# nka77/DAHiTra

Hardware: AMD Instinct MI355X
Metric: image-pairs/s (256x256) train step, 1/2/4/8 MI355X + CPU ref (higher is better)
Workload: dtype bf16; 1 GPU; LEVIR-CD 256x256 synthetic pairs, base_transformer_pos_s4, bf16, batch 32 per GPU (global 32), fwd+focal+bwd+allreduce+AdamW; net_G=base_transformer_pos_s4, global_batch=32, img_size=256, parallelism=dp1, hip_graph=True, step_form=one graph (AdamW inside), attn_dtype=bf16

## Files before the change

### dahitra_amd/csrc/conv_wgrad.hip

```cpp
#include "common.h"

namespace {

constexpr int TH = 8, TW = 16;
static inline int co_tile(int Cout) { return Cout <= 16 ? 16 : (Cout <= 32 ? 32 : 64); }

struct WgArgs {
    const void* x;
    const void* dy;
    float* part;
    int N, H, W, Cin, OH, OW, Cout, pad;
    int tilesX, tilesY, splitk, groups, npix, in_npix;
    int ci_tiles;
    int CinPitch;
    int dil;
    int CoutUse;
    int direct;
    const float* in_scale;
    const float* in_shift;
    int in_groups;
    int phase_mode;
    int no_xcd_remap;
    const void* dyt_y;
    const float* dytoef;
    int dyt_groups;
    long x_split;
};

constexpr int lds_pitch(int row_bytes) { return ((row_bytes / 32) & 1) ? row_bytes : row_bytes + 32; }

union F8 {
    s16x8 v;
    s16x4 h[2];
// ... 432 lines not shown
    bool okij[NI][4];
#pragma unroll
    for (int i = 0; i < NI; ++i)
#pragma unroll
        for (int j = 0; j < 4; ++j)
            okij[i][j] = WCI ? (cob + i * 16 + j < p.CoutUse && cib < p.Cin) : (cob + j < p.CoutUse && cib + i * 16 < p.Cin);
    if (p.direct == 2) {
#pragma unroll
        for (int t = 0; t < TAPS; ++t)
#pragma unroll
            for (int i = 0; i < NI; ++i)
#pragma unroll
                for (int j = 0; j < 4; ++j)
                    if (okij[i][j]) out[t * tstride + j * p.Cin + i * istep] += acc[t][i][j];
    } else {
#pragma unroll
        for (int t = 0; t < TAPS; ++t)
#pragma unroll
            for (int i = 0; i < NI; ++i)
#pragma unroll
                for (int j = 0; j < 4; ++j)
                    if (okij[i][j]) out[t * tstride + j * p.Cin + i * istep] = acc[t][i][j];
    }
}
template <typename T, int KS, int STRIDE, int IT, bool TR, int DIL, int CTT, int CIG, bool DYT = false>
__global__ __launch_bounds__(256 * CIG) void conv_wgrad_kernel(WgArgs p) {
    extern __shared__ __attribute__((aligned(16))) unsigned char smem[];
    wg_body<T, KS, STRIDE, IT, TR, DIL, CTT, CIG, DYT>(p, blockIdx.x, blockIdx.y, gridDim.x, gridDim.y, blockIdx.z, smem);
}
constexpr int WS_MAXJ = 16;
struct WsMulti {
    int njobs;
    int first[WS_MAXJ + 1];
    WgArgs a[WS_MAXJ];
};
static_assert(sizeof(WsMulti) <= 4096, "the kernel argument block");
template <typename T, int KS, int STRIDE, int IT, bool TR, int DIL, int CTT, int CIG>
__global__ __launch_bounds__(256 * CIG) void conv_wgrad_multi_kernel(WsMulti m) {
    extern __shared__ __attribute__((aligned(16))) unsigned char smem[];
    int j = 0;
    while (j + 1 < m.njobs && (int)blockIdx.x >= m.first[j + 1]) ++j;
    const WgArgs p = m.a[j];
    const int nbx = ((p.CoutUse + CTT - 1) / CTT) * p.ci_tiles, local = (int)blockIdx.x - m.first[j];
    if (local >= nbx * p.splitk) return;
    wg_body<T, KS, STRIDE, IT, TR, DIL, CTT, CIG, false>(p, local % nbx, local / nbx, nbx, p.splitk, 0, smem);
}

static inline int wgrad_reduce_epb(int I) { return (I & 3) == 0 ? 128 : 32; }
__device__ __forceinline__ void wgrad_reduce_block(const float* __restrict__ part, int splitk, int taps, int Oslab, int O,
                                                   int I, float* __restrict__ dw, int accumulate, long block, float (*red)[132]) {
    const long n = (long)O * I * taps;
    const int lane = threadIdx.x & 31, ph = threadIdx.x >> 5;
    const bool vec = (I & 3) == 0;
    const long i = vec ? (block * 32 + lane) * 4 : block * 32 + lane;
    float acc[4] = {0.f, 0.f, 0.f, 0.f};
    int tap = 0, ci = 0, o = 0;
    if (i < n) {
        ci = (int)(i % I);
        o = (int)((i / I) % O);
        tap = (int)(i / ((long)I * O));
        const size_t slab = (size_t)taps * Oslab * I;
        const float* src = part + ((size_t)tap * Oslab + o) * I + ci;
        if (vec) {
            float4 a0 = make_float4(0.f, 0.f, 0.f, 0.f), a1 = a0, a2 = a0, a3 = a0;
            auto add = [](float4& a, const float4 v) { a.x += v.x; a.y += v.y; a.z += v.z; a.w += v.w; };
            int k = ph;
            for (; k + 24 < splitk; k += 32) {
                add(a0, *reinterpret_cast<const float4*>(src + (size_t)k * slab));
                add(a1, *reinterpret_cast<const float4*>(src + (size_t)(k + 8) * slab));
// ... 32 lines not shown
            if (accumulate) dw[d] += s; else dw[d] = s;
        }
    }
}
__global__ void wgrad_reduce_oihw_kernel(const float* __restrict__ part, int splitk, int taps, int Oslab, int O, int I,
                                         float* __restrict__ dw, int accumulate) {
    __shared__ float red[8][132];
    const long n = (long)O * I * taps;
    wgrad_reduce_block(part + (size_t)blockIdx.y * splitk * taps * Oslab * I, splitk, taps, Oslab, O, I,
                       dw + (size_t)blockIdx.y * n, accumulate, blockIdx.x, red);
}
struct WgReduceJob {
    const float* part;
    float* dw;
    int splitk, taps, Oslab, O, I, accumulate, first_block, nblocks;
};
__global__ void wgrad_reduce_multi_kernel(const WgReduceJob* __restrict__ jobs, int njobs) {
    __shared__ float red[8][132];
    int j = 0;
    while (j + 1 < njobs && (int)blockIdx.x >= jobs[j + 1].first_block) ++j;
    const WgReduceJob job = jobs[j];
    wgrad_reduce_block(job.part, job.splitk, job.taps, job.Oslab, job.O, job.I, job.dw, job.accumulate,
                       (long)blockIdx.x - job.first_block, red);
}

#ifdef DH_WS_TIMING
__device__ long long g_ws[4096 * 16];
#define WS_NOW() ((long long)wall_clock64())
#define WS_T(...) __VA_ARGS__
#else
#define WS_T(...)
#endif
template <int DIL>
__device__ __forceinline__ void ws_body(const WgArgs& p, int bx, int kz, const int nbx, const int nkz, unsigned char* smem) {
    constexpr int KS = 3, TAPS = 9;
    constexpr int HH = (TH - 1) + (KS - 1) * DIL + 1, HWD = (TW - 1) + (KS - 1) * DIL + 1;
    constexpr int XP = lds_pitch(128), DP = lds_pitch(128);
    constexpr int STAGE = HH * HWD * XP + TH * TW * DP;
    float* bnp = reinterpret_cast<float*>(smem + 2 * STAGE);

    const int tid = threadIdx.x, lane = tid & 63, wv = tid >> 6;
    const int pl = lane & 15, g = lane >> 4;
    if (nbx > 1 && (nkz & 7) == 0 && !p.no_xcd_remap) {
        const unsigned lin = (unsigned)(kz * nbx + bx), xcd = lin & 7, sq = lin >> 3;
        bx = (int)(sq % nbx);
        kz = (int)((sq / nbx) * 8 + xcd);
    }
    const int cot = bx / p.ci_tiles, cit = bx % p.ci_tiles;
    const int co0 = cot * 64, ci0 = cit * 64;
    const int tiles_per_img = p.tilesX * p.tilesY;
    const int ntiles = p.N * tiles_per_img;
    const int my_tiles = kz < ntiles ? (ntiles - kz + p.splitk - 1) / p.splitk : 0;

    if (p.in_scale) {
        for (int i = tid; i < p.in_groups * 128; i += 512) {
            const int gi = i >> 7, k = (i >> 6) & 1, c = i & 63;
            bnp[i] = (k ? p.in_shift : p.in_scale)[gi * p.Cin + ci0 + c];
        }
        __syncthreads();
    }

    if (wv >= 4) {
        const int pt = tid - 256, q = pt & 7, prow = pt >> 3;
        constexpr int NXV = (HH * HWD + 31) / 32, NDV = TH * TW / 32;
        struct Regs { uint4 rx[NXV], rd[NDV]; unsigned okmask; int bng; };
        Regs RA, RB;
        int x_h[NXV];
#pragma unroll
        for (int i = 0; i < NXV; ++i) {
            const int px = prow + 32 * i;
            x_h[i] = px < HH * HWD ? ((px / HWD) << 8) | (px % HWD) : -1;
        }
        const unsigned xps = (unsigned)p.CinPitch * 2u, dps = (unsigned)p.Cout * 2u;
        const bool upper = p.x_split && ci0 >= p.Cin / 2;
        const long xsel = upper ? p.x_split : 0L;
        const unsigned xcb = (unsigned)((upper ? ci0 - p.Cin / 2 : ci0) + q * 8) * 2u, dcb = (unsigned)(co0 + q * 8) * 2u;
// ... 109 lines not shown
            for (int kh = 0; kh < KS; ++kh)
#pragma unroll
                for (int kw = 0; kw < KS; ++kw) {
                    const int hp = ((kk / TW) + kh * DIL) * HWD + kw * DIL;
                    F8 b;
                    b.h[0] = __builtin_amdgcn_ds_read_tr16_b64_v4i16((__attribute__((address_space(3))) s16x4*)(b_base + hp * XP));
                    b.h[1] = __builtin_amdgcn_ds_read_tr16_b64_v4i16((__attribute__((address_space(3))) s16x4*)(b_base + (hp + HWD) * XP));
#pragma unroll
                    for (int s = 0; s < 4; ++s)
                        acc[kh * KS + kw][s] = __builtin_amdgcn_mfma_f32_16x16x32_bf16(a[s].v, b.v, acc[kh * KS + kw][s], 0, 0, 0);
                }
        }
        asm volatile("s_waitcnt lgkmcnt(0)" ::: "memory");
        WS_T(tc[1] += WS_NOW() - t1;)
    }
    WS_T(const long long tloop = WS_NOW();)
    float* out = p.part + (size_t)kz * TAPS * p.Cout * p.Cin + (size_t)(co0 + g * 4) * p.Cin + ci0 + wv * 16 + pl;
    const int tstride = p.Cout * p.Cin;
#pragma unroll
    for (int t = 0; t < TAPS; ++t)
#pragma unroll
        for (int s = 0; s < 4; ++s)
#pragma unroll
            for (int j = 0; j < 4; ++j) out[t * tstride + (s * 16 + j) * p.Cin] = acc[t][s][j];
    WS_T(if (tid == 0) { long long* o = g_ws + (blockIdx.y * gridDim.x + blockIdx.x) % 4096 * 16; o[0] = tc[0]; o[1] = tc[1]; o[2] = tloop - tbeg; o[3] = WS_NOW() - tloop; o[4] = my_tiles; })
}
template <int DIL>
__global__ __launch_bounds__(512) void conv_wgrad_ws_kernel(WgArgs p) {
    extern __shared__ __attribute__((aligned(16))) unsigned char smem[];
    ws_body<DIL>(p, blockIdx.x, blockIdx.y, gridDim.x, gridDim.y, smem);
}
__global__ __launch_bounds__(512) void conv_wgrad_ws_multi_kernel(WsMulti m) {
    extern __shared__ __attribute__((aligned(16))) unsigned char smem[];
    int j = 0;
    while (j + 1 < m.njobs && (int)blockIdx.x >= m.first[j + 1]) ++j;
    const WgArgs p = m.a[j];
    const int nbx = (p.Cout / 64) * p.ci_tiles, local = (int)blockIdx.x - m.first[j];
    if (local >= nbx * p.splitk) return;
    ws_body<1>(p, local % nbx, local / nbx, nbx, p.splitk, smem);
}
#ifdef DH_WS_TIMING
extern "C" int dh_debug_ws(long long* host, int n) { return (int)hipMemcpyFromSymbol(host, HIP_SYMBOL(g_ws), (size_t)n * 8); }
#endif

enum WgFamily { WG_W1 = 0, WG_WS, WG_WS_BATCH, WG_C32_BATCH, WG_GENERIC, WG_PHASE };
enum WgPrec { WG_BF16, WG_F32, WG_X3 };
struct WgLaunch {
    int prec;
    bool tr;
    int ks, stride, accumulate;
    bool batch;
};
struct WgPlan {
    int family;
    int it, ct, cig, ci_tiles;
    int splitk, direct, threads;
    dim3 grid;
    size_t lds;
};

constexpr size_t ws_lds(int dil, int in_groups) {
    return 2 * ((size_t)((TH - 1) + 2 * dil + 1) * ((TW - 1) + 2 * dil + 1) * lds_pitch(128) + (size_t)TH * TW * lds_pitch(128)) +
           (size_t)in_groups * 128 * sizeof(float);
}
constexpr size_t wg_lds(int ks, int stride, int dil, int it, int ct, int cig, int le, int npl, int in_groups, int dyt_groups) {
    const int hh = (TH - 1) * stride + (ks - 1) * dil + 1, hw = (TW - 1) * stride + (ks - 1) * dil + 1;
    const size_t lds = npl * ((size_t)hh * hw * lds_pitch(it * cig * le) + (size_t)TH * TW * lds_pitch(ct * le)) +
                       (size_t)in_groups * 2 * it * cig * sizeof(float) + (size_t)dyt_groups * 3 * ct * sizeof(float);
    const size_t red = ct < 64 ? (size_t)(ct / 16) * ks * ks * (it / 16) * 64 * 16 : 0;
    return lds < red ? red : lds;
}
template <typename K>
// ... 17 lines not shown
}

struct WsBatch {
    int ct, n;
    size_t lds;
    bool on;
    WsMulti m;
};
static thread_local WsBatch g_wsb{64, 0, 0, false};
static thread_local WsBatch g_c32b{32, 0, 0, false};
static int batch_splitk(long tiles, int tpw, int cap) {
    long sk = tiles / (tpw > 0 ? tpw : 32);
    if (sk > cap) sk = cap;
    if (sk >= 8) sk &= ~7L;
    return (int)(sk < 1 ? 1 : sk);
}
static int batch_tpw(int ct, int blocks) {
    static const int tpw = getenv("DAHITRA_WGRAD_TPW") ? atoi(getenv("DAHITRA_WGRAD_TPW")) : 32;
    static const int tpw_big = getenv("DAHITRA_WGRAD_TPW_BIG") ? atoi(getenv("DAHITRA_WGRAD_TPW_BIG")) : 2 * tpw;
    static const int tpw32 = getenv("DAHITRA_WGRAD_TPW32") ? atoi(getenv("DAHITRA_WGRAD_TPW32")) : 32;
    return ct == 32 ? tpw32 : (blocks >= 16 ? tpw_big : tpw);
}
static void batch_sort(WsBatch& b) {
    auto tpw = [](const WgArgs& a) { return ((long)a.N * a.tilesX * a.tilesY + a.splitk - 1) / a.splitk; };
    const int n = getenv("DAHITRA_WGRAD_NO_SORT") ? 0 : b.n;
    for (int i = 1; i < n; ++i)
        for (int j = i; j > 0 && tpw(b.m.a[j]) > tpw(b.m.a[j - 1]); --j) { const WgArgs t = b.m.a[j]; b.m.a[j] = b.m.a[j - 1]; b.m.a[j - 1] = t; }
    b.m.first[0] = 0;
    for (int i = 0; i < b.n; ++i) {
        const int nblocks = dh_cdiv(b.m.a[i].CoutUse, b.ct) * b.m.a[i].ci_tiles * b.m.a[i].splitk;
        b.m.first[i + 1] = b.m.first[i] + ((nblocks + 7) & ~7);
    }
}
static int batch_flush(WsBatch& b, hipStream_t st) {
    if (b.n == 0) return 0;
    b.m.njobs = b.n;
    batch_sort(b);
    const bool ws = b.ct == 64;
    static size_t raised_ws = 0, raised_c32 = 64 * 1024;
    const char* name = ws ? "conv_wgrad_ws_multi" : "conv_wgrad_multi";
    auto kern = ws ? conv_wgrad_ws_multi_kernel : conv_wgrad_multi_kernel<bf16, 3, 1, 32, true, 1, 32, 1>;
    if (const int rc = raise_dynamic_lds(kern, ws ? ws_lds(1, 8) : b.lds, ws ? raised_ws : raised_c32, name)) return rc;
    hipLaunchKernelGGL(kern, dim3(b.m.first[b.n]), dim3(ws ? 512 : 256), b.lds, st, b.m);
    b.n = 0; b.lds = 0;
    DH_CHECK_LAUNCH(name);
    return 0;
}
static int batch_add(WsBatch& b, const WgArgs& a, size_t lds, hipStream_t st) {
    if (b.n == WS_MAXJ) { const int rc = batch_flush(b, st); if (rc) return rc; }
    b.m.a[b.n++] = a;
    if (lds > b.lds) b.lds = lds;
    return 0;
}

template <typename T, int KS, int STRIDE, int IT, int DIL, int CT, int CIG = 1>
int launch_ct(const WgArgs& a, const WgPlan& p, bool tr, hipStream_t st) {
    auto go = [&](auto kern) -> int {
        static size_t raised = 64 * 1024;
        if (const int rc = raise_dynamic_lds(kern, p.lds, raised, "conv_wgrad")) return rc;
        hipLaunchKernelGGL(kern, p.grid, dim3(p.threads), p.lds, st, a);
        DH_CHECK_LAUNCH("conv_wgrad");
        return 0;
    };
    if constexpr (KS == 4 && CT == 64 && sizeof(T) == 2) {
        if (a.dyt_y) {
            if (tr) return go(conv_wgrad_kernel<T, KS, STRIDE, IT, true, DIL, CT, CIG, true>);
            return go(conv_wgrad_kernel<T, KS, STRIDE, IT, false, DIL, CT, CIG, true>);
        }
    }
    if (a.dyt_y) DH_FAIL("conv_wgrad: the BatchNorm-backward-on-load form is built for the bf16 stem (4x4, 64 output channels)");
    if constexpr (Prec<T>::X3) return go(conv_wgrad_kernel<T, KS, STRIDE, IT, true, DIL, CT, CIG>);
    else {
        if (tr) return go(conv_wgrad_kernel<T, KS, STRIDE, IT, true, DIL, CT, CIG>);
        return go(conv_wgrad_kernel<T, KS, STRIDE, IT, false, DIL, CT, CIG>);
    }
}
// ... 299 lines not shown
    WgArgs a = wg_args(N, H, W, Cin, OH, OW, Cout, pad);
    a.x = x; a.dy = dy; a.x_split = x_split; a.dil = dilation; a.groups = groups; a.phase_mode = phase;
    a.dyt_y = dyt_y; a.dytoef = dytoef; a.dyt_groups = dyt_groups;
    a.in_scale = in_scale; a.in_shift = in_shift; a.in_groups = in_groups > 0 ? in_groups : 1;
    if (in_scale) DH_REQUIRE(in_shift && groups == 1 && N % a.in_groups == 0 && (Cin * (dtype == DH_DTYPE_BF16 ? 2 : 4)) % 16 == 0,
                             "conv2d_wgrad: BatchNorm-on-load needs in_shift, one weight group, N %% in_groups == 0, 16-byte channel pieces");
    if (cin_pitch > 0) a.CinPitch = cin_pitch;
    if (Cout_real > 0) a.CoutUse = Cout_real;
    if (npix_valid > 0) a.npix = a.in_npix = npix_valid;
    const int prec = dtype == DH_DTYPE_BF16 ? WG_BF16 : (wgrad_x3(dtype, a) ? WG_X3 : WG_F32);
    const bool batch = describe ? batch_open != 0 : (g_wsb.on && defer);
    const WgLaunch l{prec, prec == WG_BF16 ? use_tr != 0 : prec == WG_X3, ks, stride, accumulate, batch};
    WgPlan p;
    const int e = wg_plan(a, l, p);
    if (e == WG_NO_SPLIT) DH_FAIL("conv2d_wgrad: a split input is served by the wave-specialised 3x3 kernel only (Cin=%d Cout=%d ks=%d)", Cin, Cout, ks);
    if (e == WG_NO_KERNEL) DH_FAIL("conv_wgrad: unsupported kernel %d stride %d", ks, stride);
    if (describe) {
        const int v[12] = {p.family, p.ct, p.it, p.cig, p.ci_tiles, p.splitk, p.direct, (int)p.grid.x, (int)p.grid.y, (int)p.grid.z, p.threads, (int)p.lds};
        memcpy(describe, v, sizeof(v));
        return 0;
    }
    a.part = a.direct ? dw_oihw : reinterpret_cast<float*>(workspace);
    hipStream_t st = reinterpret_cast<hipStream_t>(stream);
    if (const int rc = wg_launch(a, l, p, st)) return rc;
    if (splitk_out) *splitk_out = a.direct ? 0 : a.splitk;
    if (a.direct || defer) return 0;
    const long n = (long)a.CoutUse * Cin * ks * ks;
    hipLaunchKernelGGL(wgrad_reduce_oihw_kernel, dim3(dh_cdiv(n, wgrad_reduce_epb(Cin)), groups), dim3(256), 0, st, a.part, a.splitk,
                       ks * ks, Cout, a.CoutUse, Cin, dw_oihw, accumulate);
    DH_CHECK_LAUNCH("wgrad_reduce");
    return 0;
}

extern "C" int dh_wgrad_batch_begin() { g_wsb.on = true; g_wsb.n = 0; g_wsb.lds = 0; g_c32b.n = 0; g_c32b.lds = 0; return 0; }
extern "C" int dh_wgrad_batch_pending() { return g_wsb.n + g_c32b.n; }
extern "C" int dh_wgrad_batch_abort() { g_wsb.on = false; g_wsb.n = 0; g_wsb.lds = 0; g_c32b.n = 0; g_c32b.lds = 0; return 0; }
extern "C" int dh_wgrad_batch_launch(void* stream) {
    const int rc = batch_flush(g_wsb, reinterpret_cast<hipStream_t>(stream));
    return rc ? rc : batch_flush(g_c32b, reinterpret_cast<hipStream_t>(stream));
}
extern "C" int dh_wgrad_batch_end(void* stream) {
    const int rc = dh_wgrad_batch_launch(stream);
    g_wsb.on = false;
    return rc;
}

extern "C" int dh_conv2d_wgrad(int dtype, const void* x, const void* dy, float* dw_oihw, int accumulate, int N,
                               int H, int W, int Cin, int OH, int OW, int Cout, int ks, int stride, int pad,
                               int groups, int npix_valid, int use_tr, int Cout_real, int cin_pitch, int dilation,
                               void* workspace, void* stream) {
    return conv2d_wgrad_impl(dtype, x, dy, dw_oihw, accumulate, N, H, W, Cin, OH, OW, Cout, ks, stride, pad, groups,
                             npix_valid, use_tr, Cout_real, cin_pitch, dilation, workspace, stream, 0, nullptr);
}

extern "C" int dh_conv2d_wgrad_partial(int dtype, const void* x, const void* dy, float* dw_oihw, int accumulate, int N,
                                       int H, int W, int Cin, int OH, int OW, int Cout, int ks, int stride, int pad,
                                       int groups, int npix_valid, int use_tr, int Cout_real, int cin_pitch,
                                       int dilation, void* workspace, int* splitk_out, void* stream) {
    DH_REQUIRE(groups == 1 && splitk_out, "conv2d_wgrad_partial: one group only");
    return conv2d_wgrad_impl(dtype, x, dy, dw_oihw, accumulate, N, H, W, Cin, OH, OW, Cout, ks, stride, pad, groups,
                             npix_valid, use_tr, Cout_real, cin_pitch, dilation, workspace, stream, 1, splitk_out);
}
bool dh_wgrad_split_supported(int N, int H, int W, int Cin, int Cout) {
    WgArgs a = wg_args(N, H, W, Cin, H, W, Cout, 1);
    a.CinPitch = Cin / 2; a.x_split = 16;
    WgPlan p;
    return wg_plan(a, WgLaunch{WG_BF16, true, 3, 1, 0, false}, p) == WG_OK && p.family == WG_WS;
}
extern "C" int dh_conv2d_wgrad_split(const void* x, long x_split_bytes, const void* dy, float* dw_oihw, int accumulate, int N, int H,
// ... 163 lines not shown
```

### dahitra_amd/ops.py

```python
import bisect
import ctypes
import math
import os
import sys

import numpy as np
import torch

from . import _lib

ACT_NONE, ACT_RELU, ACT_GELU = 0, 1, 2
_DT = {torch.float32: 0, torch.bfloat16: 1}
_vp = ctypes.c_void_p


def dt(t):
    try:
        return _DT[t.dtype]
    except KeyError:
        raise TypeError("dahitra_amd: unsupported activation dtype %s" % t.dtype)


def set_f32_mma_mode(mode):
    _lib.check(_lib.lib().dh_set_f32_mma_mode(int(mode)), "dh_set_f32_mma_mode")
# ... 133 lines not shown
        nb = max(1, min(256, cdiv(n, 2048)))
        if ks == 3 and O % 32 == 0 and I % 32 == 0 and OK == O:
            nb = min(256, (O // 32) * (I // 32))
        self.jobs.append(self._Job(w.data_ptr(), fwd.data_ptr() if fwd is not None else None,
                                   dg.data_ptr() if dg is not None else None, O, I, ks, OPad, IPad, OK,
                                   _DT[dtype] | (0x200 if frag else 0), self.blocks, nb))
        self.blocks += nb
        self.keep += [w, fwd, dg]
        return fwd, dg

    def run(self):
        if not self.jobs:
            return
        if self.table is None:
            assert ctypes.sizeof(self._Job) == _lib.lib().dh_pack_job_size()
            raw = b"".join(bytes(j) for j in self.jobs)
            self.table = torch.frombuffer(bytearray(raw), dtype=torch.uint8).to(self.device)
        _call("dh_pack_weights_multi", P(self.table), len(self.jobs), self.blocks, S())


class WgradPlan:

    class _Job(ctypes.Structure):
        _fields_ = [("part", ctypes.c_void_p), ("dw", ctypes.c_void_p), ("splitk", ctypes.c_int), ("taps", ctypes.c_int),
                    ("Oslab", ctypes.c_int), ("O", ctypes.c_int), ("I", ctypes.c_int), ("accumulate", ctypes.c_int),
                    ("first_block", ctypes.c_int), ("nblocks", ctypes.c_int)]

    def __init__(self, device, batch=False):
        self.device, self.slots, self.cur, self.blocks = device, [], 0, 0
        self.tables, self.sigs, self.phase = {}, {}, 0
        self._prev = None
        self.post = []
        self.batch = batch and os.environ.get("DAHITRA_WGRAD_BATCH", "1") != "0"
        self.batching, self.keep = False, []

    def __enter__(self):
        global _WGRAD_PLAN
        self._prev, _WGRAD_PLAN = _WGRAD_PLAN, self
        self.cur = 0
        self.jobs = []
        self.post = []
        self.blocks = 0
        self.phase = 0
        self.keep = []
        self.batching = self.batch and PROFILE is None
        if self.batching:
            _call("dh_wgrad_batch_begin")
        elif self._prev is None:
            _call("dh_wgrad_batch_abort")
        return self

    def __exit__(self, *exc):
        global _WGRAD_PLAN
        _WGRAD_PLAN = self._prev
        if self.batching:
            self.batching = False
            if exc and exc[0] is not None:
                _lib.lib().dh_wgrad_batch_abort()
            else:
                _call("dh_wgrad_batch_end", S())
            self.keep = []
        return False

    def hold(self, *tensors):
        if self.batching:
            self.keep += [t for t in tensors if t is not None]

    def slab(self, nbytes):
        if self.cur == len(self.slots):
            self.slots.append(torch.empty(max(int(nbytes), 16), dtype=torch.uint8, device=self.device))
        elif self.slots[self.cur].numel() < nbytes:
            _PINNED.append(self.slots[self.cur])
            self.slots[self.cur] = torch.empty(int(nbytes), dtype=torch.uint8, device=self.device)
            self.tables = {}
        buf = self.slots[self.cur]
        self.cur += 1
        return buf

    def add(self, part, dw, splitk, taps, oslab, o, i, accumulate):
        nb = cdiv(o * i * taps, _lib.lib().dh_wgrad_reduce_outputs_per_block(i))
        self.jobs.append(self._Job(part.data_ptr(), dw.data_ptr(), splitk, taps, oslab, o, i, int(accumulate),
                                   self.blocks, nb))
        self.blocks += nb

    def run(self):
        if self.batching:
            _call("dh_wgrad_batch_launch", S())
            self.keep = []
        if self.jobs:
            self._run_reduce()
        for fn in self.post:
            fn()
        self.jobs, self.post, self.blocks = [], [], 0
        self.phase += 1

    def _run_reduce(self):
        sig = b"".join(bytes(j) for j in self.jobs)
        if self.tables.get(self.phase) is None or sig != self.sigs.get(self.phase):
            if torch.cuda.is_current_stream_capturing():
                raise RuntimeError("dahitra_amd: the weight-gradient plan changed during graph capture; run one eager "
                                   "step of the same shapes first")
            assert ctypes.sizeof(self._Job) == _lib.lib().dh_wgrad_reduce_job_size()
            if self.tables.get(self.phase) is not None:
                _PINNED.append(self.tables[self.phase])
            self.tables[self.phase] = torch.frombuffer(bytearray(sig), dtype=torch.uint8).to(self.device)
            self.sigs[self.phase] = sig
        _call("dh_wgrad_reduce_multi", P(self.tables[self.phase]), len(self.jobs), self.blocks, S())


_WGRAD_PLAN = None


class SideStream:

    def __init__(self, device):
        self.stream, self.keep, self.active, self._ctx = torch.cuda.Stream(device=device), [], False, None

    def fork(self, *tensors):
        global _PERSIST_BLOCK
        self.stream.wait_stream(torch.cuda.current_stream())
        self.keep += [t for t in tensors if t is not None]
        if not self.active:
            _PERSIST_BLOCK += 1
        self.active = True
        return self

    def __enter__(self):
# ... 2022 lines not shown
```

### include/dahitra_hip.h

```cpp
#ifndef DAHITRA_HIP_H
#define DAHITRA_HIP_H
#ifdef __cplusplus
extern "C" {
#endif

#define DH_F32 0
#define DH_BF16 1
#define DH_ACT_NONE 0
#define DH_ACT_RELU 1
#define DH_ACT_GELU 2

int dh_abi_version(void);
const char* dh_last_error(void);
void dh_set_error(const char* msg);

int dh_conv2d_fwd(int dtype, const void* x, const void* w_packed, void* y, const float* bias,
                  const void* residual, float* stats_partial, int N, int H, int W, int Cin, int OH, int OW,
                  int Cout, int CoutPad, int ks, int stride, int pad, int act, int npix_valid,
                  long w_image_stride, void* y_preact, int dilation, const void* gate_out, const void* gate_y,
                  const float* gate_mean, const float* gate_invstd, int gate_groups, const float* in_scale,
                  const float* in_shift, int in_groups, int phase_mode, const void* w_frag, void* stream);
int dh_conv2d_fwd_num_tiles(int dtype, int N, int OH, int OW, int Cin, int ks, int stride);
int dh_conv2d_fwd_describe(int entry, int dtype, int N, int H, int W, int Cin, int OH, int OW, int Cout, int CoutPad, int ks, int stride,
                           int pad, int act, int npix_valid, long w_image_stride, int dilation, int gate_groups, int in_groups,
// ... 8 lines not shown
int dh_conv3x3_dgrad_up4(int dtype, const void* dy, const void* w_packed, int N, int H, int W, int K, float* partial, void* stream);
int dh_absdiff_up4_combine(const float* partial, const void* a, const void* b, void* da, void* db, int N, int H, int W, void* stream);
int dh_conv3x3_head_fwd(int dtype, const void* x, const void* w_packed, const float* bias, int N, int H, int W, int Cin,
                        int Cout, const float* in_scale, const float* in_shift, int in_groups, float* logits_nchw, void* stream);

int dh_conv2d_wgrad(int dtype, const void* x, const void* dy, float* dw_oihw, int accumulate, int N, int H,
                    int W, int Cin, int OH, int OW, int Cout, int ks, int stride, int pad, int groups,
                    int npix_valid, int use_tr, int Cout_real, int cin_pitch, int dilation, void* workspace, void* stream);
int dh_conv2d_wgrad_1x1_blocks(int N, int H, int W, int Cin, int Cout);
int dh_conv2d_wgrad_describe(int dtype, int accumulate, int N, int H, int W, int Cin, int OH, int OW, int Cout, int ks, int stride,
                             int pad, int groups, int npix_valid, int use_tr, int Cout_real, int cin_pitch, int dilation,
                             int in_groups, int has_in_scale, int split_input, int batch_open, int* out);
long dh_conv2d_wgrad_workspace_size(int N, int OH, int OW, int Cin, int Cout, int ks, int groups);
int dh_conv2d_wgrad_partial(int dtype, const void* x, const void* dy, float* dw_oihw, int accumulate, int N, int H,
                            int W, int Cin, int OH, int OW, int Cout, int ks, int stride, int pad, int groups,
                            int npix_valid, int use_tr, int Cout_real, int cin_pitch, int dilation, void* workspace,
                            int* splitk_out, void* stream);
int dh_conv2d_wgrad_bn_in(int dtype, const void* x, const void* dy, float* dw_oihw, int accumulate, int N, int H, int W,
                          int Cin, int OH, int OW, int Cout, int ks, int stride, int pad, int use_tr, int Cout_real,
                          int dilation, const float* in_scale, const float* in_shift, int in_groups, void* workspace,
                          int* splitk_out, void* stream);
int dh_conv3x3_split_supported(int N, int H, int W, int Cin, int Cout);
int dh_conv3x3_split_fwd(const void* x, long x_split_bytes, const void* w_packed, const void* w_frag, void* y, long y_split_bytes,
                         float* stats_partial, int N, int H, int W, int Cin, int Cout, void* stream);
int dh_conv2d_wgrad_split(const void* x, long x_split_bytes, const void* dy, float* dw_oihw, int accumulate, int N, int H, int W,
                          int Cin, int Cout, void* workspace, int* splitk_out, void* stream);
int dh_conv3x3_up4_fwd(const void* a, const void* b, const void* w_packed, const float* bias, int act, void* y, float* stats_partial,
                       int N, int H, int W, void* stream);
int dh_wgrad_batch_begin(void);
int dh_wgrad_batch_pending(void);
int dh_wgrad_batch_launch(void* stream);
int dh_wgrad_batch_end(void* stream);
int dh_wgrad_batch_abort(void);
int dh_wgrad_reduce_multi(const void* jobs_dev, int njobs, int total_blocks, void* stream);
int dh_pack_phase_weights(int dtype, const float* w_oihw, const float* bias, int Cin, void* fwd, void* dgrad, float* bias4,
                          void* stream);
long dh_conv2d_wgrad_phase_workspace_size(int N, int H, int W, int Cin);
int dh_conv2d_wgrad_phase(int dtype, const void* x, const void* dy, int N, int H, int W, int Cin, int use_tr, void* workspace,
                          int* splitk_out, void* stream);
int dh_phase_wgrad_combine(const float* dwab, float* dw_oihw, int Cin, int accumulate, void* stream);
int dh_pack_s2_dgrad_phase_weights(int dtype, const float* w_oihw, int Co, int Ci, void* out, void* stream);
int dh_wgrad_reduce_job_size(void);
int dh_wgrad_reduce_outputs_per_block(int Cin);
int dh_conv2d_wgrad_splitk(int N, int OH, int OW, int Cin, int Cout, int ks, int groups);

int dh_pack_weight(int dtype, const float* w_oihw, const float* out_scale, int O, int I, int ks, int OPad, void* fwd, int IPad,
                   int dgrad_inner, void* dgrad, void* stream);
int dh_pack_weights_multi(const void* jobs_dev, int njobs, int total_blocks, void* stream);
int dh_pack_job_size(void);
int dh_zero_insert2(int dtype, const void* dy, void* z, int N, int OH, int OW, int H, int W, int C, void* stream);
int dh_add_coarse(int dtype, void* x, const void* coarse, int N, int OH, int OW, int H, int W, int C, void* stream);

int dh_stem_space_to_depth(int dtype, const float* x_nchw, void* y, int N, int H, int W, int CP, void* stream);
int dh_stem_pack_weight(int dtype, const float* w_oihw, const float* out_scale, void* packed, int O, int CP, void* stream);
int dh_stem_unpack_grad(const float* dw2, float* dw_oihw, int O, int CP, int accumulate, void* stream);
int dh_stem7_fwd(const float* xa, const float* xb, int B, int N, int H, int W, const float* w_oihw, const float* out_scale,
                 const float* bias, int relu, void* y, float* stats, int groups, void* xs16, void* stream);
int dh_stem7_fwd_num_slots(int N, int H, int W, int groups);
long dh_stem_pool_bn_bwd_workspace_size(int C, int groups);
int dh_stem_pool_bn_bwd(const unsigned char* argmax, const void* dpool, const void* y, const float* mask_scale,
                        const float* mask_shift, const float* mean, const float* invstd, const float* gamma, int N, int H, int W,
                        int C, int groups, void* d, float* coef, float* dgamma, float* dbeta, int accumulate, void* workspace,
                        void* stream);
int dh_stem_pool_bn_bwd_plus(const unsigned char* argmax, const void* dpool, const void* extra, const void* y,
                             const float* mask_scale, const float* mask_shift, const float* mean, const float* invstd,
                             const float* gamma, int N, int H, int W, int C, int groups, void* d, float* coef, float* dgamma,
// ... 308 lines not shown
```

Baseline: 9795 image-pairs/s.

## Balance batched wgrad split-K slices across XCDs with a makespan-driven planner

Adds a host-side planner for the batched 3x3 wgrad multi-kernel. It searches per-layer split-K counts and can assign workgroup slots per XCD, using a simulated makespan over the device's CUs to pick the layout. The chosen split counts are sent back to Python so the reduce jobs use matching slices. The intent is to cut tail imbalance across layers and XCDs, at the cost of host planning (memoized) and more kernel-argument state.

```diff
diff --git a/dahitra_amd/csrc/conv_wgrad.hip b/dahitra_amd/csrc/conv_wgrad.hip
--- a/dahitra_amd/csrc/conv_wgrad.hip
+++ b/dahitra_amd/csrc/conv_wgrad.hip
@@ -1,4 +1,7 @@
 #include "common.h"
+#include <algorithm>
+#include <utility>
+#include <vector>
 
 namespace {
 
@@ -497,9 +500,35 @@
 struct WsMulti {
     int njobs;
     int first[WS_MAXJ + 1];
+    int slots;
+    unsigned short off[WS_MAXJ + 1][8];
+    unsigned short kbase[WS_MAXJ][8];
     WgArgs a[WS_MAXJ];
 };
 static_assert(sizeof(WsMulti) <= 4096, "the kernel argument block");
+__host__ __device__ inline bool ws_map(const WsMulti& m, int w, int& j, int& bx, int& kz) {
+    j = 0;
+    if (m.slots) {
+        const int x = w & 7, slot = w >> 3;
+        if (slot >= (int)m.off[m.njobs][x]) return false;
+        while (j + 1 < m.njobs && slot >= (int)m.off[j + 1][x]) ++j;
+        const int nbx = (m.a[j].Cout / 64) * m.a[j].ci_tiles, q = slot - (int)m.off[j][x];
+        bx = q % nbx;
+        kz = (int)m.kbase[j][x] + q / nbx;
+        return true;
+    }
+    while (j + 1 < m.njobs && w >= m.first[j + 1]) ++j;
+    const int nbx = (m.a[j].Cout / 64) * m.a[j].ci_tiles, nkz = m.a[j].splitk, local = w - m.first[j];
+    if (local >= nbx * nkz) return false;
+    bx = local % nbx;
+    kz = local / nbx;
+    if (nbx > 1 && (nkz & 7) == 0 && !m.a[j].no_xcd_remap) {
+        const unsigned xcd = (unsigned)local & 7, sq = (unsigned)local >> 3;
+        bx = (int)(sq % nbx);
+        kz = (int)((sq / nbx) * 8 + xcd);
+    }
+    return true;
+}
 template <typename T, int KS, int STRIDE, int IT, bool TR, int DIL, int CTT, int CIG>
 __global__ __launch_bounds__(256 * CIG) void conv_wgrad_multi_kernel(WsMulti m) {
     extern __shared__ __attribute__((aligned(16))) unsigned char smem[];
@@ -598,7 +627,8 @@
 #define WS_T(...)
 #endif
 template <int DIL>
-__device__ __forceinline__ void ws_body(const WgArgs& p, int bx, int kz, const int nbx, const int nkz, unsigned char* smem) {
+__device__ __forceinline__ void ws_body(const WgArgs& p, int bx, int kz, const int nbx, const int nkz, unsigned char* smem,
+                                        const bool remap = true) {
     constexpr int KS = 3, TAPS = 9;
     constexpr int HH = (TH - 1) + (KS - 1) * DIL + 1, HWD = (TW - 1) + (KS - 1) * DIL + 1;
     constexpr int XP = lds_pitch(128), DP = lds_pitch(128);
@@ -607,7 +637,7 @@
 
     const int tid = threadIdx.x, lane = tid & 63, wv = tid >> 6;
     const int pl = lane & 15, g = lane >> 4;
-    if (nbx > 1 && (nkz & 7) == 0 && !p.no_xcd_remap) {
+    if (remap && nbx > 1 && (nkz & 7) == 0 && !p.no_xcd_remap) {
         const unsigned lin = (unsigned)(kz * nbx + bx), xcd = lin & 7, sq = lin >> 3;
         bx = (int)(sq % nbx);
         kz = (int)((sq / nbx) * 8 + xcd);
@@ -783,12 +813,10 @@
 }
 __global__ __launch_bounds__(512) void conv_wgrad_ws_multi_kernel(WsMulti m) {
     extern __shared__ __attribute__((aligned(16))) unsigned char smem[];
-    int j = 0;
-    while (j + 1 < m.njobs && (int)blockIdx.x >= m.first[j + 1]) ++j;
+    int j, bx, kz;
+    if (!ws_map(m, (int)blockIdx.x, j, bx, kz)) return;
     const WgArgs p = m.a[j];
-    const int nbx = (p.Cout / 64) * p.ci_tiles, local = (int)blockIdx.x - m.first[j];
-    if (local >= nbx * p.splitk) return;
-    ws_body<1>(p, local % nbx, local / nbx, nbx, p.splitk, smem);
+    ws_body<1>(p, bx, kz, (p.Cout / 64) * p.ci_tiles, p.splitk, smem, false);
 }
 #ifdef DH_WS_TIMING
 extern "C" int dh_debug_ws(long long* host, int n) { return (int)hipMemcpyFromSymbol(host, HIP_SYMBOL(g_ws), (size_t)n * 8); }
@@ -872,16 +900,173 @@
         b.m.first[i + 1] = b.m.first[i] + ((nblocks + 7) & ~7);
     }
 }
+
+constexpr int WS_TURN = 4;
+static int g_balance_cus = 0;
+static inline int ws_nbx(const WgArgs& a) { return (a.Cout / 64) * a.ci_tiles; }
+static inline long ws_tiles(const WgArgs& a) { return (long)a.N * a.tilesX * a.tilesY; }
+static int ws_layout(WsMulti& m, const int* slices, bool xcd_slots, int* order) {
+    const int n = m.njobs;
+    for (int i = 0; i < n; ++i) { m.a[i].splitk = slices[i]; order[i] = i; }
+    auto tpw = [](const WgArgs& a) { return (ws_tiles(a) + a.splitk - 1) / a.splitk; };
+    static const bool no_sort = getenv("DAHITRA_WGRAD_NO_SORT") != nullptr;
+    for (int i = 1; i < (no_sort ? 0 : n); ++i)
+        for (int j = i; j > 0 && tpw(m.a[j]) > tpw(m.a[j - 1]); --j) {
+            const WgArgs t = m.a[j]; m.a[j] = m.a[j - 1]; m.a[j - 1] = t;
+            const int o = order[j]; order[j] = order[j - 1]; order[j - 1] = o;
+        }
+    m.first[0] = 0;
+    for (int i = 0; i < n; ++i) m.first[i + 1] = m.first[i] + ((ws_nbx(m.a[i]) * m.a[i].splitk + 7) & ~7);
+    m.slots = xcd_slots ? 1 : 0;
+    if (!xcd_slots) return m.first[n];
+    long work[8] = {0};
+    int end[8] = {0}, cnt[WS_MAXJ][8] = {}, heavy[WS_MAXJ];
+    auto gcost = [&](int j) { return (long)ws_nbx(m.a[j]) * (tpw(m.a[j]) + WS_TURN); };
+    for (int i = 0; i < n; ++i) {
+        heavy[i] = i;
+        for (int j = i; j > 0 && gcost(heavy[j]) > gcost(heavy[j - 1]); --j) { const int o = heavy[j]; heavy[j] = heavy[j - 1]; heavy[j - 1] = o; }
+    }
+    for (int i = 0; i < n; ++i) {
+        const int j = heavy[i];
+        for (int k = 0; k < m.a[j].splitk; ++k) {
+            int x = 0;
+            for (int y = 1; y < 8; ++y) if (work[y] < work[x]) x = y;
+            ++cnt[j][x]; work[x] += gcost(j);
+        }
+    }
+    for (int j = 0; j < n; ++j)
+        for (int x = 0, k = 0; x < 8; ++x) {
+            if (end[x] > 0xffff || k > 0xffff) return 0;
+            m.off[j][x] = (unsigned short)end[x]; m.kbase[j][x] = (unsigned short)k;
+            end[x] += cnt[j][x] * ws_nbx(m.a[j]); k += cnt[j][x];
+        }
+    int most = 0;
+    for (int x = 0; x < 8; ++x) {
+        if (end[x] > 0xffff) return 0;
+        m.off[n][x] = (unsigned short)end[x];
+        if (end[x] > most) most = end[x];
+    }
+    return most * 8;
+}
+static long ws_makespan(const WsMulti& m, int grid, int cus) {
+    constexpr int MAXC = 64;
+    long free_at[8][MAXC] = {};
+    int ncu[8];
+    for (int x = 0; x < 8; ++x) { ncu[x] = cus / 8 + (x < cus % 8 ? 1 : 0); if (ncu[x] < 1) ncu[x] = 1; if (ncu[x] > MAXC) ncu[x] = MAXC; }
+    long span = 0;
+    for (int w = 0; w < grid; ++w) {
+        int j, bx, kz;
+        if (!ws_map(m, w, j, bx, kz)) continue;
+        const long tiles = ws_tiles(m.a[j]), s = m.a[j].splitk;
+        const long cost = (kz < tiles ? (tiles - kz + s - 1) / s : 0) + WS_TURN;
+        const int x = w & 7;
+        int c = 0;
+        for (int d = 1; d < ncu[x]; ++d) if (free_at[x][d] < free_at[x][c]) c = d;
+        free_at[x][c] += cost;
+        if (free_at[x][c] > span) span = free_at[x][c];
+    }
+    return span;
+}
+static int ws_balance(WsMulti& m, int cus, bool balance, int* order, long* info) {
+    const int n = m.njobs;
+    int rec[WS_MAXJ], best[WS_MAXJ], cur[WS_MAXJ], prev[WS_MAXJ] = {0}, ord[WS_MAXJ];
+    for (int i = 0; i < n; ++i) rec[i] = m.a[i].splitk;
+    WsMulti t = m;
+    const long rec_span = ws_makespan(t, ws_layout(t, rec, false, ord), cus);
+    long best_span = -1;
+    bool best_slots = false;
+    const bool slots_ok = balance && !m.a[0].no_xcd_remap;
+    bool wide = !slots_ok;
+    for (int i = 0; i < n; ++i) wide = wide || ws_nbx(m.a[i]) > cus / 8;
+    auto consider = [&](const int* s) {
+        for (int form = slots_ok ? 1 : 0; form >= (wide ? 0 : 1); --form) {
+            t = m;
+            const int grid = ws_layout(t, s, form != 0, ord);
+            if (!grid) continue;
+            const long span = ws_makespan(t, grid, cus);
+            if (best_span < 0 || span < best_span) { best_span = span; best_slots = form != 0; memcpy(best, s, sizeof(best)); }
+        }
+    };
+    if (balance) {
+        std::vector<long> cand;
+        for (int i = 0; i < n; ++i)
+            for (int s = 1; s <= rec[i]; ++s) cand.push_back((ws_tiles(m.a[i]) + s - 1) / s);
+        std::sort(cand.begin(), cand.end(), [](long a, long b) { return a > b; });
+        cand.erase(std::unique(cand.begin(), cand.end()), cand.end());
+        for (const long L : cand) {
+            bool same = true;
+            for (int i = 0; i < n; ++i) {
+                const long s = (ws_tiles(m.a[i]) + L - 1) / L;
+                cur[i] = (int)(s > rec[i] ? rec[i] : (s < 1 ? 1 : s));
+                same = same && cur[i] == prev[i];
+            }
+            if (same) continue;
+            memcpy(prev, cur, sizeof(cur));
+            consider(cur);
+        }
+        consider(rec);
+    }
+    const bool take = best_span >= 0 && best_span <= rec_span;
+    const int grid = ws_layout(m, take ? best : rec, take && best_slots, order);
+    if (info) { info[0] = m.slots; info[1] = take ? best_span : rec_span; info[2] = rec_span; }
+    return grid;
+}
+struct WsPlanMemo { std::vector<long> key; int slices[WS_MAXJ]; bool slots; };
+static int ws_balance_cached(WsMulti& m, int cus, int* order) {
+    static thread_local WsPlanMemo memo[4];
+    static thread_local int next = 0;
+    std::vector<long> key{cus};
+    for (int i = 0; i < m.njobs; ++i)
+        for (const long v : {(long)ws_nbx(m.a[i]), ws_tiles(m.a[i]), (long)m.a[i].splitk, (long)m.a[i].no_xcd_remap}) key.push_back(v);
+    for (const WsPlanMemo& e : memo)
+        if (e.key == key) return ws_layout(m, e.slices, e.slots, order);
+    WsPlanMemo& e = memo[next++ & 3];
+    const int grid = ws_balance(m, cus, true, order, nullptr);
+    for (int i = 0; i < m.njobs; ++i) e.slices[order[i]] = m.a[i].splitk;
+    e.slots = m.slots != 0;
+    e.key = key;
+    return grid;
+}
+static int balance_cus() {
+    if (g_balance_cus > 0) return g_balance_cus;
+    static int cus = 0;
+    if (cus <= 0) {
+        int dev = 0, v = 0;
+        if (hipGetDevice(&dev) != hipSuccess || hipDeviceGetAttribute(&v, hipDeviceAttributeMultiprocessorCount, dev) != hipSuccess || v <= 0) {
+            (void)hipGetLastError();
+            return 0;
+        }
+        cus = v;
+    }
+    return cus;
+}
+static thread_local std::vector<std::pair<const void*, int>> g_issued;
+
 static int batch_flush(WsBatch& b, hipStream_t st) {
     if (b.n == 0) return 0;
     b.m.njobs = b.n;
-    batch_sort(b);
+    b.m.slots = 0;
     const bool ws = b.ct == 64;
+    static const bool balance = !(getenv("DAHITRA_WGRAD_BALANCE") && atoi(getenv("DAHITRA_WGRAD_BALANCE")) == 0);
+    int grid = 0;
+    if (ws && balance) {
+        const int cus = balance_cus();
+        if (cus <= 0) DH_FAIL("conv_wgrad_ws_multi: cannot read the device's CU count");
+        int order[WS_MAXJ];
+        std::pair<const void*, int> rec[WS_MAXJ];
+        grid = ws_balance_cached(b.m, cus, order);
+        for (int i = 0; i < b.n; ++i) rec[order[i]] = {b.m.a[i].part, b.m.a[i].splitk};
+        g_issued.insert(g_issued.end(), rec, rec + b.n);
+    } else {
+        for (int i = 0; i < b.n; ++i) g_issued.push_back({b.m.a[i].part, b.m.a[i].splitk});
+        batch_sort(b);
+        grid = b.m.first[b.n];
+    }
     static size_t raised_ws = 0, raised_c32 = 64 * 1024;
     const char* name = ws ? "conv_wgrad_ws_multi" : "conv_wgrad_multi";
     auto kern = ws ? conv_wgrad_ws_multi_kernel : conv_wgrad_multi_kernel<bf16, 3, 1, 32, true, 1, 32, 1>;
     if (const int rc = raise_dynamic_lds(kern, ws ? ws_lds(1, 8) : b.lds, ws ? raised_ws : raised_c32, name)) return rc;
-    hipLaunchKernelGGL(kern, dim3(b.m.first[b.n]), dim3(ws ? 512 : 256), b.lds, st, b.m);
+    hipLaunchKernelGGL(kern, dim3(grid), dim3(ws ? 512 : 256), b.lds, st, b.m);
     b.n = 0; b.lds = 0;
     DH_CHECK_LAUNCH(name);
     return 0;
@@ -1247,9 +1432,43 @@
     return 0;
 }
 
-extern "C" int dh_wgrad_batch_begin() { g_wsb.on = true; g_wsb.n = 0; g_wsb.lds = 0; g_c32b.n = 0; g_c32b.lds = 0; return 0; }
+extern "C" int dh_wgrad_batch_begin() { g_wsb.on = true; g_wsb.n = 0; g_wsb.lds = 0; g_c32b.n = 0; g_c32b.lds = 0; g_issued.clear(); return 0; }
 extern "C" int dh_wgrad_batch_pending() { return g_wsb.n + g_c32b.n; }
-extern "C" int dh_wgrad_batch_abort() { g_wsb.on = false; g_wsb.n = 0; g_wsb.lds = 0; g_c32b.n = 0; g_c32b.lds = 0; return 0; }
+extern "C" int dh_wgrad_batch_abort() { g_wsb.on = false; g_wsb.n = 0; g_wsb.lds = 0; g_c32b.n = 0; g_c32b.lds = 0; g_issued.clear(); return 0; }
+extern "C" int dh_wgrad_batch_issued(int cap, void** workspaces, int* slices) {
+    const int n = (int)g_issued.size();
+    DH_REQUIRE(n == 0 || (n <= cap && workspaces && slices), "wgrad_batch_issued: %d layers issued, room for %d", n, cap);
+    for (int i = 0; i < n; ++i) { workspaces[i] = const_cast<void*>(g_issued[i].first); slices[i] = g_issued[i].second; }
+    g_issued.clear();
+    return n;
+}
+extern "C" int dh_wgrad_balance_set_cus(int cus) { g_balance_cus = cus > 0 ? cus : 0; return 0; }
+extern "C" int dh_wgrad_balance_describe(int njobs, const int* blocks, const int* tiles, const int* recorded, int cus, int balance,
+                                         int* slices, int* info, int* map, int map_cap) {
+    DH_REQUIRE(njobs >= 1 && njobs <= WS_MAXJ && blocks && tiles && recorded && cus > 0 && slices && info,
+               "wgrad_balance_describe: bad arguments (njobs=%d cus=%d)", njobs, cus);
+    WsMulti m{};
+    m.njobs = njobs;
+    for (int i = 0; i < njobs; ++i) {
+        DH_REQUIRE(blocks[i] >= 1 && tiles[i] >= 1 && recorded[i] >= 1, "wgrad_balance_describe: layer %d is empty", i);
+        WgArgs& a = m.a[i];
+        a.N = tiles[i]; a.tilesX = a.tilesY = 1; a.Cout = 64 * blocks[i]; a.ci_tiles = 1; a.splitk = recorded[i];
+    }
+    int order[WS_MAXJ];
+    long span[3];
+    const int grid = ws_balance(m, cus, balance != 0, order, span);
+    for (int i = 0; i < njobs; ++i) slices[order[i]] = m.a[i].splitk;
+    info[0] = grid; info[1] = (int)span[0]; info[2] = (int)span[1]; info[3] = (int)span[2];
+    if (map) {
+        DH_REQUIRE(map_cap >= grid, "wgrad_balance_describe: %d workgroups, room for %d", grid, map_cap);
+        for (int w = 0; w < grid; ++w) {
+            int j, bx, kz;
+            const bool on = ws_map(m, w, j, bx, kz);
+            map[3 * w] = on ? order[j] : -1; map[3 * w + 1] = on ? bx : -1; map[3 * w + 2] = on ? kz : -1;
+        }
+    }
+    return 0;
+}
 extern "C" int dh_wgrad_batch_launch(void* stream) {
     const int rc = batch_flush(g_wsb, reinterpret_cast<hipStream_t>(stream));
     return rc ? rc : batch_flush(g_c32b, reinterpret_cast<hipStream_t>(stream));
diff --git a/dahitra_amd/ops.py b/dahitra_amd/ops.py
--- a/dahitra_amd/ops.py
+++ b/dahitra_amd/ops.py
@@ -189,7 +189,7 @@
         self._prev = None
         self.post = []
         self.batch = batch and os.environ.get("DAHITRA_WGRAD_BATCH", "1") != "0"
-        self.batching, self.keep = False, []
+        self.batching, self.keep, self.issued = False, [], []
 
     def __enter__(self):
         global _WGRAD_PLAN
@@ -244,12 +244,23 @@
         if self.batching:
             _call("dh_wgrad_batch_launch", S())
             self.keep = []
+            self._take_issued_slices()
         if self.jobs:
             self._run_reduce()
         for fn in self.post:
             fn()
         self.jobs, self.post, self.blocks = [], [], 0
         self.phase += 1
+
+    def _take_issued_slices(self):
+        cap = max(len(self.jobs), 1)
+        parts, slices = (ctypes.c_void_p * cap)(), (ctypes.c_int * cap)()
+        n = _lib.lib().dh_wgrad_batch_issued(cap, parts, slices)
+        _lib.check(0 if n >= 0 else n, "dh_wgrad_batch_issued")
+        self.issued = [slices[i] for i in range(n)]
+        took = {parts[i]: slices[i] for i in range(n)}
+        for job in self.jobs:
+            job.splitk = took.get(job.part, job.splitk)
 
     def _run_reduce(self):
         sig = b"".join(bytes(j) for j in self.jobs)
diff --git a/include/dahitra_hip.h b/include/dahitra_hip.h
--- a/include/dahitra_hip.h
+++ b/include/dahitra_hip.h
@@ -64,6 +64,10 @@
 int dh_wgrad_batch_launch(void* stream);
 int dh_wgrad_batch_end(void* stream);
 int dh_wgrad_batch_abort(void);
+int dh_wgrad_batch_issued(int cap, void** workspaces, int* slices);
+int dh_wgrad_balance_set_cus(int cus);
+int dh_wgrad_balance_describe(int njobs, const int* blocks, const int* tiles, const int* recorded, int cus, int balance,
+                              int* slices, int* info, int* map, int map_cap);
 int dh_wgrad_reduce_multi(const void* jobs_dev, int njobs, int total_blocks, void* stream);
 int dh_pack_phase_weights(int dtype, const float* w_oihw, const float* bias, int Cin, void* fwd, void* dgrad, float* bias4,
                           void* stream);
```

Measured after the change: 9780 image-pairs/s. No clear change (-0.2%).
